# JaehaKim97/EDTR

Hardware: AMD Instinct MI355X
Metric: restored 512x512 images/sec @ 4 denoise steps (higher is better)
Workload: dtype bf16; 1 GPU; EDTR-det s4 (sd21): vae_encode + q_sample(t=200) + 4 x (ControlNet+UNet) + vae_decode, batch 8/GPU of 512x512; global_batch=8, image_size=512, denoise_steps=4, parallelism=batch-sharded x1, graphs=True, batches_in_flight=2, precision=fast

## Files before the change

### edtr_amd/build.py

```python
from __future__ import annotations

import os
import shutil
import subprocess
import sys

HERE = os.path.dirname(os.path.abspath(__file__))
CSRC = os.path.join(HERE, "csrc")
LIB_PATH = os.path.join(HERE, "libedtr_hip.so")
SOURCES = ["igemm.hip", "halo512.hip", "attention.hip", "attn512.hip", "norm.hip", "elementwise.hip", "swin.hip", "ffn.hip", "lin320.hip"]
HEADERS = [os.path.join(CSRC, "common.h"), os.path.join(os.path.dirname(HERE), "include", "edtr_hip.h")]
EXTRA_DEPS = {"attention.hip": [os.path.join(CSRC, "attn_v3_loop.inc")]}
ARCH = "gfx950"


def _hipcc() -> str:
    for cand in (os.environ.get("HIPCC"), shutil.which("hipcc"), "/opt/rocm/bin/hipcc"):
        if cand and os.path.exists(cand):
            return cand
    raise RuntimeError("hipcc not found (needed to build libedtr_hip.so)")


def _stale(target: str, deps) -> bool:
    if not os.path.exists(target):
        return True
    t = os.path.getmtime(target)
    return any(os.path.getmtime(d) > t for d in deps)


def source_hash() -> str:
    import hashlib
    h = hashlib.sha1()
    files = sorted(f for f in os.listdir(CSRC) if f.endswith((".hip", ".inc", ".h")))
# ... 62 lines not shown
```

### edtr_amd/engine.py

```python
from __future__ import annotations

import collections
import ctypes as ct
import math
import os
from dataclasses import dataclass
from typing import Dict, List, Optional, Sequence, Tuple

import torch

from . import lib as L
from . import ops
from .ops import Rec, round_up


class Arena:

    ALIGN = 256

    def __init__(self, device: torch.device, chunk_bytes: int = 1 << 28):
        self.device = device
        self.chunk_bytes = chunk_bytes
        self.chunks: List[torch.Tensor] = []
        self.free_lists: List[List[List[int]]] = []
# ... 235 lines not shown
            w1p, b1p, c1, c2 = self.ln_fold("geglu", [w1name], [b1name], ln_prefix)
            cst = ops.pack_ffn_constants(c2 + b1p)
            w2p = ops.pack_ffn_w2(self._p(w2name).reshape(self.params[w2name].shape[0], -1), self.dtype)
            self.cache[key] = (w1p, w2p, cst, self._p(b2name).reshape(-1).contiguous())
        return self.cache[key]

    def lin320(self, names: Sequence[str], biases, ln_prefix: Optional[str], alpha: float, vt_col0: Optional[int] = None, vt_alpha: float = 1.0):
        names = tuple(names)
        key = ("lin320", names, tuple(biases) if biases else None, ln_prefix, float(alpha), vt_col0, float(vt_alpha))
        if key not in self.cache:
            w = torch.cat([self._p(n).reshape(self.params[n].shape[0], -1) for n in names], dim=0)
            cvec = None
            if biases:
                cvec = torch.cat([self._p(bn).reshape(-1) if bn else torch.zeros(self.params[n].shape[0], device=self.device)
                                  for n, bn in zip(names, biases)]).float()
            if ln_prefix is not None:
                gamma, beta = self._p(ln_prefix + "weight").reshape(-1), self._p(ln_prefix + "bias").reshape(-1)
                shift = float(alpha) * (w @ beta)
                if vt_col0 is not None:
                    shift[vt_col0:] *= float(vt_alpha) / float(alpha)
                cvec = shift if cvec is None else cvec + shift
                w = w * gamma[None, :]
            self.cache[key] = (ops.pack_lin320_w(w, self.dtype), cvec.contiguous() if cvec is not None else None)
        return self.cache[key]

    def raw(self, name: str) -> torch.Tensor:
        key = ("raw", name)
        if key not in self.cache:
            self.cache[key] = self._p(name).contiguous()
        return self.cache[key]

    def geglu(self, wname: str, bname: str):
        n, k = self.shape_of(wname)[0], self.shape_of(wname)[1]

        def build(parts):
            w = self._p(wname)
            perm = ops.geglu_perm(w.shape[0] // 2).to(self.device)
            return ops.pack_linear_weight(w[perm], self.dtype, parts=parts)

        ref = WRef(self, ("geglu", wname), build, (round_up(n, 8), round_up(k, 8)))
        key = ("geglu.bias", bname)
        if key not in self.cache:
            b = self._p(bname)
            self.cache[key] = b[ops.geglu_perm(b.shape[0] // 2).to(self.device)].contiguous()
        return ref, self.cache[key]

# ... 305 lines not shown
        y = self.arena.alloc((rows, C), dtype or self.attn_dtype)
        self.prog.add(ops.make_cast16(dtype=dtype or self.attn_dtype, src=x, rows=rows, C=C, dst=y))
        return y

    @staticmethod
    def _w(w, parts: int) -> torch.Tensor:
        return w.get(parts) if isinstance(w, WRef) else w

    def ln_fold_ok(self, C: int, B: int = 0) -> bool:
        if self.hp or C % 32 or self.invariant:
            return False
        mode = os.environ.get("EDTR_LN_FOLD", "auto")
        if mode in ("0", "1"):
            return mode == "1"
        return 0 < B <= ops.LN_FOLD_MAX_BATCH

    def _ln_kwargs(self, a, K: int, ln_vec):
        if a.C != K or ln_vec is None:
            raise ValueError("folded LayerNorm: the consumer needs K == C and the folded weight's (c1, c2)")
        return a.x, dict(ln_stats=a.stats, ln_C=a.C, ln_valid=a.c_valid, ln_eps=1e-5, ln_c1=ln_vec[0], ln_c2=ln_vec[1])

    def ffn_ok(self, rows: int, C: int) -> bool:
        return not self.hp and not self.invariant and ops.ffn_ok(rows, C, 4 * C)

    def lin320_ok(self, rows: int, N: int, K: int, ln: bool = False) -> bool:
        return not self.hp and not self.invariant and ops.lin320_ok(rows, N, K, ln)

    def lin320(self, x: torch.Tensor, rows: int, N: int, names, biases=None, *, ln_prefix: Optional[str] = None, alpha: float = 1.0,
               residual: Optional[torch.Tensor] = None, gn_table: Optional[torch.Tensor] = None, rows_per_image: int = 0,
               name: str = "lin320") -> torch.Tensor:
        self.last_gnp, self.last_row_stats, self.gnp_into_done = None, None, False
        w, cvec = self.store.lin320(names, biases, ln_prefix, alpha)
        out = self.new(rows, N)
        self.prog.add(ops.make_lin320(dtype=self.dtype, x=x, ldx=x.stride(0), M=rows, N=N, w=w, cvec=cvec, alpha=alpha, ln=ln_prefix is not None,
                                      eps=1e-5, residual=residual, ldr=residual.stride(0) if residual is not None else 0, out=out,
                                      ldo=out.stride(0), gn_table=gn_table, rows_per_image=rows_per_image, name=name))
        return out

    def qkv_lin320(self, x: torch.Tensor, names, *, B: int, N: int, C: int, ln_prefix: str, alpha: float, name: str = "attn1.qkv"):
        M = B * N
        w, cvec = self.store.lin320(names, None, ln_prefix, alpha, vt_col0=2 * C, vt_alpha=1.0)
        qk = self.arena.alloc((M, 2 * C), self.attn_dtype)
        vt = self.arena.alloc((B * C, N), self.attn_dtype)
        self.prog.add(ops.make_lin320(dtype=self.dtype, x=x, ldx=x.stride(0), M=M, N=3 * C, w=w, cvec=cvec, alpha=alpha, ln=True, eps=1e-5, out=qk,
                                      ldo=2 * C, vt_out=vt, vt_col0=2 * C, vt_ld=N, vt_alpha=1.0, rows_per_image=N, name=name))
        return qk, vt, N
# ... 459 lines not shown
```

### edtr_amd/lib.py

```python
from __future__ import annotations

import ctypes as C
import os
from typing import Optional

HERE = os.path.dirname(os.path.abspath(__file__))
LIB_PATH = os.environ.get("EDTR_AMD_LIB") or os.path.join(HERE, "libedtr_hip.so")

BF16, F16, F32_SPLIT, F32_H1, F32_H2, F32_H3 = 0, 1, 2, 3, 4, 5
ACT_NONE, ACT_GEGLU, ACT_SILU, ACT_GELU, ACT_LRELU = 0, 1, 2, 3, 4

DECLARED_SYMBOLS = [
    "edtr_abi_version", "edtr_error_string", "edtr_device_info", "edtr_igemm", "edtr_flash_attn64",
    "edtr_gn_stats", "edtr_gn_apply", "edtr_gn_finalize", "edtr_gn_table", "edtr_layernorm", "edtr_softmax_rows", "edtr_nchw_to_nhwc",
    "edtr_nhwc_to_nchw", "edtr_add", "edtr_timestep_embedding", "edtr_sampler_update", "edtr_axpby", "edtr_q_sample", "edtr_split3", "edtr_cast16",
    "edtr_tile_accumulate", "edtr_divide", "edtr_wavelet_level", "edtr_gn_pool", "edtr_copy3d_f32", "edtr_graph_begin", "edtr_graph_end", "edtr_graph_launch",
    "edtr_graph_destroy", "edtr_zero_bytes", "edtr_embed_tokens", "edtr_window_attn", "edtr_pixel_unshuffle", "edtr_swin_mlp", "edtr_swin_attn", "edtr_swin_layer", "edtr_conv64", "edtr_conv128_out",
    "edtr_split_operand", "edtr_sampler_update_indexed", "edtr_gaussian_sample", "edtr_add_mirror", "edtr_igemm_plan", "edtr_flash_attn512",
    "edtr_ffn", "edtr_ffn_plan", "edtr_add_stats", "edtr_lin320", "edtr_lin320_plan",
]


class IgemmParams(C.Structure):
    _fields_ = [
        ("dtype", C.c_int32), ("taps", C.c_int32), ("M", C.c_int32), ("N", C.c_int32), ("K", C.c_int32),
        ("n_valid", C.c_int32), ("Z", C.c_int32), ("zdiv", C.c_int32),
        ("a1", C.c_void_p), ("a2", C.c_void_p),
        ("C1", C.c_int32), ("C2", C.c_int32), ("ld1", C.c_int32), ("ld2", C.c_int32),
        ("a_zs_outer", C.c_int64), ("a_zs_inner", C.c_int64),
        ("IH", C.c_int32), ("IW", C.c_int32), ("OH", C.c_int32), ("OW", C.c_int32),
        ("stride", C.c_int32), ("pad_t", C.c_int32), ("pad_l", C.c_int32), ("upsample2x", C.c_int32),
        ("w", C.c_void_p), ("ldw", C.c_int32),
        ("w_zs_outer", C.c_int64), ("w_zs_inner", C.c_int64),
        ("alpha", C.c_float),
        ("bias_n", C.c_void_p), ("bias_m", C.c_void_p),
        ("rowvec", C.c_void_p), ("rowvec_ld", C.c_int32), ("rows_per_image", C.c_int32),
        ("act", C.c_int32),
        ("residual", C.c_void_p), ("ldr", C.c_int32),
        ("out", C.c_void_p), ("ldc", C.c_int32), ("out_f32", C.c_int32),
        ("o_zs_outer", C.c_int64), ("o_zs_inner", C.c_int64),
        ("tile", C.c_int32), ("splitk", C.c_int32),
        ("workspace", C.c_void_p), ("workspace_bytes", C.c_int64),
# ... 52 lines not shown


class FfnParams(C.Structure):
    _fields_ = [
        ("dtype", C.c_int32), ("M", C.c_int32), ("D", C.c_int32), ("H", C.c_int32),
        ("eps", C.c_float),
        ("x", C.c_void_p), ("ldx", C.c_int32),
        ("w1", C.c_void_p), ("w2", C.c_void_p),
        ("cst", C.c_void_p), ("b2", C.c_void_p),
        ("out", C.c_void_p), ("ldo", C.c_int32),
    ]


class Lin320Params(C.Structure):
    _fields_ = [
        ("dtype", C.c_int32), ("M", C.c_int32), ("N", C.c_int32), ("K", C.c_int32),
        ("ln", C.c_int32), ("eps", C.c_float), ("alpha", C.c_float),
        ("x", C.c_void_p), ("ldx", C.c_int32),
        ("w", C.c_void_p), ("cvec", C.c_void_p),
        ("residual", C.c_void_p), ("ldr", C.c_int32),
        ("out", C.c_void_p), ("ldo", C.c_int32),
        ("vt_out", C.c_void_p), ("vt_col0", C.c_int32), ("vt_ld", C.c_int32), ("vt_alpha", C.c_float), ("rows_per_image", C.c_int32),
        ("gn_table", C.c_void_p),
    ]


class SwinAttnParams(C.Structure):
    _fields_ = [
        ("dtype", C.c_int32), ("B", C.c_int32), ("H", C.c_int32), ("W", C.c_int32),
        ("heads", C.c_int32), ("head_dim", C.c_int32), ("shift", C.c_int32),
        ("C", C.c_int32), ("c_valid", C.c_int32),
        ("eps", C.c_float),
        ("x", C.c_void_p), ("ldx", C.c_int32),
        ("wqkv", C.c_void_p), ("wproj", C.c_void_p),
        ("c1", C.c_void_p), ("c2b", C.c_void_p), ("bproj", C.c_void_p),
        ("bias", C.c_void_p), ("labels", C.c_void_p),
        ("out", C.c_void_p), ("ldo", C.c_int32),
    ]


class Conv64Params(C.Structure):
    _fields_ = [
        ("dtype", C.c_int32), ("B", C.c_int32), ("H", C.c_int32), ("W", C.c_int32),
        ("upsample2x", C.c_int32),
        ("x", C.c_void_p), ("ldx", C.c_int32),
        ("w", C.c_void_p), ("bias", C.c_void_p),
# ... 74 lines not shown
    lib.edtr_copy3d_f32.argtypes = [vp, i64, i64, vp, i64, i64, i32, i32, i32, vp]
    lib.edtr_graph_begin.argtypes = [vp]
    lib.edtr_graph_end.argtypes = [vp, C.POINTER(vp)]
    lib.edtr_graph_launch.argtypes = [vp, vp]
    lib.edtr_graph_destroy.argtypes = [vp]
    for name in DECLARED_SYMBOLS:
        fn = getattr(lib, name)
        if name not in ("edtr_error_string",):
            fn.restype = i32
    lib.edtr_zero_bytes.argtypes = [vp, i64, vp]
    lib.edtr_embed_tokens.argtypes = [i32, vp, vp, vp, i32, i32, i32, i32, vp, i32, vp]
    lib.edtr_window_attn.argtypes = [C.POINTER(WindowAttnParams), vp]
    lib.edtr_pixel_unshuffle.argtypes = [i32, vp, i32, i32, i32, i32, i32, vp, f32, vp, i32, i32, vp]
    lib.edtr_swin_mlp.argtypes = [C.POINTER(SwinMlpParams), vp]
    lib.edtr_swin_attn.argtypes = [C.POINTER(SwinAttnParams), vp]
    lib.edtr_conv64.argtypes = [C.POINTER(Conv64Params), vp]
    lib.edtr_conv128_out.argtypes = [C.POINTER(Conv128OutParams), vp]
    lib.edtr_swin_layer.argtypes = [C.POINTER(SwinAttnParams), C.POINTER(SwinMlpParams), vp]
    lib.edtr_add_stats.argtypes = [i32, vp, i32, vp, i32, vp, i32, i64, i32, vp, i32, i32, vp]
    lib.edtr_ffn.argtypes = [C.POINTER(FfnParams), vp]
    lib.edtr_ffn_plan.argtypes = [C.POINTER(FfnParams)]
    lib.edtr_lin320.argtypes = [C.POINTER(Lin320Params), vp]
    lib.edtr_lin320_plan.argtypes = [C.POINTER(Lin320Params)]
    if lib.edtr_abi_version() != 10:
        raise RuntimeError("libedtr_hip.so ABI version mismatch")
    _lib = lib
    return lib


def check(code: int, what: str = "") -> None:
    if code != 0:
        msg = load().edtr_error_string(code).decode()
        raise RuntimeError(f"libedtr_hip {what} failed with code {code}: {msg}")
```

### edtr_amd/model/cldm.py

```python
from __future__ import annotations

import os
from typing import Dict, List, Optional, Set, Tuple

import torch
from torch import nn

from .. import arch, nets
from .. import ops as ops_mod
from ..engine import Act, Arena, Emitter, EngineCache, Program, WeightStore
from .clip import FrozenOpenCLIPEmbedder
from .params import ParamTree, params_fingerprint

_DTYPES = {"bf16": torch.bfloat16, "bfloat16": torch.bfloat16, "fp16": torch.float16, "float16": torch.float16}


def default_compute_dtype() -> torch.dtype:
    return _DTYPES[os.environ.get("EDTR_AMD_DTYPE", "bf16").lower()]


PRECISIONS = ("fast", "mixed", "high", "hybrid", "robust")

HYBRID_SECTIONS = {"cldm": "fast16", "vae.encode": "fast16", "vae.decode": "mixed"}
_SECTION_MODES = {"fast16": ("fast", torch.float16), "fastbf16": ("fast", torch.bfloat16), "mixed": ("mixed", None), "high": ("high", None)}
# ... 152 lines not shown


class CldmEngine:

    def __init__(self, owner: "ControlLDM", B: int, h: int, w: int, nctx: int):
        dev = owner._device()
        mode, dt = section_mode(owner.precision, owner.compute_dtype, "cldm")
        pol = _policy_for(owner, "cldm")
        self.B, self.h, self.w, self.nctx = B, h, w, nctx
        self.arena = Arena(dev)
        store = owner._store("cldm")
        ua, ca = owner.unet.arch, owner.controlnet.arch
        f32 = torch.float32
        self.x_in = torch.zeros((B, ua.in_channels, h, w), dtype=f32, device=dev)
        self.hint_in = torch.zeros((B, ca.hint_channels, h, w), dtype=f32, device=dev)
        self.t_in = torch.zeros((B,), dtype=torch.int64, device=dev)
        self.ctx_in = torch.zeros((B, nctx, ua.context_dim), dtype=f32, device=dev)
        self.eps_out = torch.zeros((B, ua.out_channels, h, w), dtype=f32, device=dev)
        self.ctx_key = None

        self.ctx_prog = Program("cldm.context")
        em = Emitter(self.ctx_prog, self.arena, store, dt, mode, pol)
        ctx16 = em.cast_flat(self.ctx_in, B * nctx * ua.context_dim).view(B * nctx, ua.context_dim)
        self.kv_c = nets.emit_context_kv(em, "controlnet.", ca, ctx16, B, nctx)
        self.kv_u = nets.emit_context_kv(em, "unet.", ua, ctx16, B, nctx)

        self.step_prog = Program("cldm.step")
        em = Emitter(self.step_prog, self.arena, store, dt, mode, pol)
        hw = h * w
        cin_c = ca.in_channels + ca.hint_channels
        x8c = em.new(B * hw, arch_round8(cin_c))
        em.to_nhwc(self.x_in, B, ca.in_channels, hw, x8c, coff=0)
        em.to_nhwc(self.hint_in, B, ca.hint_channels, hw, x8c, coff=ca.in_channels,
                   pad_to=arch_round8(cin_c) - ca.in_channels)
        x8u = em.new(B * hw, arch_round8(ua.in_channels))
        em.to_nhwc(self.x_in, B, ua.in_channels, hw, x8u, coff=0, pad_to=arch_round8(ua.in_channels))
        tab_c, offs_c = nets.emit_time_rows(em, "controlnet.", ca, self.t_in, B)
        tab_u, offs_u = nets.emit_time_rows(em, "unet.", ua, self.t_in, B)
        self.arena_cn = Arena(dev)
        em_cn = Emitter(self.step_prog, self.arena_cn, store, dt, mode, pol)
        self.step_prog.fork()
        self.step_prog.set_lane(1)
        ctrl = nets.emit_controlnet(em_cn, "controlnet.", ca, Act(x8c, B, h, w, x8c.shape[1]), tab_c, offs_c, self.kv_c,
                                    list(owner.control_scales))
        self.step_prog.set_lane(0)
        eps = nets.emit_unet(em, "unet.", ua, Act(x8u, B, h, w, x8u.shape[1]), tab_u, offs_u, self.kv_u, ctrl,
                             before_control=self.step_prog.join)
        em.to_nchw(eps, B, ua.out_channels, hw, self.eps_out)
# ... 377 lines not shown
```

### edtr_amd/nets.py

```python
from __future__ import annotations

import math
import os
from typing import Dict, List, Optional, Tuple

import torch

from . import lib as L
from . import ops
from .arch import Layer, UNetArch, VaeLayer
from .engine import Act, Emitter, LNRef, LNReg
from .ops import round_up


def emit_time_rows(em: Emitter, P: str, a: UNetArch, t_dev: torch.Tensor, B: int) -> Tuple[torch.Tensor, Dict[str, int]]:
    mc, ted = a.model_channels, a.model_channels * 4
    temb = em.new(B, mc)
    em.prog.add(ops.make_timestep_embedding(dtype=em.io, t=t_dev, B=B, dim=mc, out=temb, ld=mc))
    w0, b0 = em.store.linear([P + "time_embed.0.weight"], [P + "time_embed.0.bias"])
    h = em.gemm(temb, w0, B, ted, mc, bias=b0, act=L.ACT_SILU, name="time_embed.0")
    w2, b2 = em.store.linear([P + "time_embed.2.weight"], [P + "time_embed.2.bias"])
    semb = em.gemm(h, w2, B, ted, ted, bias=b2, act=L.ACT_SILU, name="time_embed.2")
    res = a.res_layers()
    wall, ball = em.store.linear([P + l.prefix + "emb_layers.1.weight" for l in res],
# ... 1 lines not shown
    total = wall.shape[0]
    table = em.gemm(semb, wall, B, total, ted, bias=ball, out_f32=True, name="emb_layers(all)")
    em.free(temb, h, semb)
    offs, o = {}, 0
    for l in res:
        offs[l.prefix] = o
        o += l.cout
    return table, offs


ATTN_PRESCALE = 1.4426950408889634 / math.sqrt(64.0)


class ContextKV:

    def __init__(self):
        self.k_all = None
        self.vt_all = None
        self.sumC = 0
        self.ldv = 0
        self.Nctx = 0
        self.split = 0
        self.offs: Dict[str, int] = {}


def emit_context_kv(em: Emitter, P: str, a: UNetArch, ctx16: torch.Tensor, B: int, Nctx: int) -> ContextKV:
    layers = a.attn_layers()
    kv = ContextKV()
    t = "transformer_blocks.0.attn2."
    wk, _ = em.store.linear([P + l.prefix + t + "to_k.weight" for l in layers])
    wv, _ = em.store.linear([P + l.prefix + t + "to_v.weight" for l in layers])
    kv.sumC, kv.Nctx = wk.shape[0], Nctx
    kv.split = em.attn_split
    kv.k_all = em.gemm(ctx16, wk, B * Nctx, kv.sumC, a.context_dim, name="ctx_k(all)", out16=kv.split < 1)
    kv.vt_all, kv.ldv = em.vt_gemm(wv, ctx16, B=B, Ntok=Nctx, Cin=a.context_dim, name="ctx_vT(all)", out16=kv.split < 2)
    if kv.k_all.dtype == torch.float32:
        k32 = kv.k_all
        kv.k_all = em.split16(k32, B * Nctx, kv.sumC) if kv.split >= 1 else em.to16(k32, B * Nctx, kv.sumC)
        em.free(k32)
    if kv.vt_all.dtype == torch.float32:
        v32 = kv.vt_all
        kv.vt_all = em.split16(v32, B * kv.sumC, kv.ldv) if kv.split >= 2 else em.to16(v32, B * kv.sumC, kv.ldv)
        em.free(v32)
    o = 0
    for l in layers:
        kv.offs[l.prefix] = o
        o += l.cout
    return kv


def emit_resblock(em: Emitter, P: str, l: Layer, x: Act, table: torch.Tensor, offs: Dict[str, int], out=None, mirror=False, gnp_into=None) -> Act:
    p = P + l.prefix
    n1 = em.group_norm(x, p + "in_layers.0.", 1e-5, True, feeds=("res.conv1",), conv_n=l.cout)
    h = em.conv(n1, p + "in_layers.2.", rowvec=table[:, offs[l.prefix]:], name="res.conv1", stats=True, feeds=("res.conv2",))
    em.free(n1)
    n2 = em.group_norm(h, p + "out_layers.0.", 1e-5, True, feeds=("res.conv2",), conv_n=l.cout, take=True)
    em.free(h)
    if l.cin != l.cout:
        skip = em.conv(x, p + "skip_connection.", taps=1, name="res.skip1x1").t
    else:
        skip = x.t
    y = em.conv(n2, p + "out_layers.3.", residual=skip, out=out, name="res.conv2", stats=out is None, mirror=mirror, gnp_into=gnp_into)
    into_done = em.gnp_into_done
    em.free(n2)
    if l.cin != l.cout:
        em.free(skip)
    em.gnp_into_done = into_done
    return y


# ... 59 lines not shown
        t = em.gemm(n.t, wi, rows, C, C, bias=bi, name="st.proj_in", row_stats=fold1)
    st = em.last_row_stats
    em.free(n)
    tb = p + "transformer_blocks.0."
    if (st is None and em.fused_qkv_ok(N, C) and em.lin320_ok(rows, 3 * C, C, ln=True) and N % 32 == 0 and em.attn_dtype == em.dtype
            and os.environ.get("EDTR_LIN320_QKV", "1") != "0"):
        l1 = LNReg(t, C, tb + "norm1.")
    else:
        l1 = em.layer_norm(t, rows, C, tb + "norm1.", feeds=("attn1.qkv",) if em.fused_qkv_ok(N, C) else ("attn1.qk", "attn1.vT"), stats=st)
    t1 = emit_attention_core(em, tb + "attn1.", l1, B, N, C, l.heads, None, t, row_stats=fold)
    st = em.last_row_stats
    em.free(l1, t)
    l2 = (LNReg(t1, C, tb + "norm2.") if (st is None and em.lin320_ok(rows, C, C, ln=True))
          else em.layer_norm(t1, rows, C, tb + "norm2.", feeds=("attn2.q",), stats=st))
    off = kv.offs[l.prefix]
    k_view = kv.k_all[:, off:off + C]
    k_lo = kv.k_all[:, kv.sumC + off:kv.sumC + off + C] if kv.split >= 1 else None
    ldv_all = kv.vt_all.stride(0)
    vt3 = kv.vt_all.view(B, kv.sumC, ldv_all)
    vt_view = vt3[:, off:off + C, :kv.ldv]
    vt_lo = vt3[:, off:off + C, kv.ldv:] if kv.split >= 2 else None
    ctx = (k_view, vt_view, kv.Nctx * kv.k_all.stride(0), kv.sumC * ldv_all, ldv_all, kv.Nctx, k_lo, vt_lo)
    fused_ff = em.ffn_ok(rows, C)
    t2 = emit_attention_core(em, tb + "attn2.", l2, B, N, C, l.heads, ctx, t1, row_stats=fold and not fused_ff)
    st = em.last_row_stats
    em.free(l2, t1)
    if fused_ff:
        t3 = em.ffn(t2, rows, C, tb)
        em.free(t2)
    else:
        l3 = em.layer_norm(t2, rows, C, tb + "norm3.", feeds=("ff.geglu",), stats=st)
        if isinstance(l3, LNRef):
            wg, bg, c1, c2 = em.store.ln_fold("geglu", [tb + "ff.net.0.proj.weight"], [tb + "ff.net.0.proj.bias"], l3.prefix)
            g = em.gemm(l3, wg, rows, 8 * C, C, bias=bg, act=L.ACT_GEGLU, name="ff.geglu", feeds="ff.out", ln_vec=(c1, c2))
        else:
            wg, bg = em.store.geglu(tb + "ff.net.0.proj.weight", tb + "ff.net.0.proj.bias")
            g = em.gemm(l3, wg, rows, 8 * C, C, bias=bg, act=L.ACT_GEGLU, name="ff.geglu", feeds="ff.out")
        em.free(l3)
        wf, bf = em.store.linear([tb + "ff.net.2.weight"], [tb + "ff.net.2.bias"])
        t3 = em.gemm(g, wf, rows, C, 4 * C, bias=bf, residual=t2, name="ff.out", feeds="st.proj_out" if em.branch16 else None)
        em.free(g, t2)
    wo, bo = em.store.linear([p + "proj_out.weight"], [p + "proj_out.bias"])
    y = em.gemm(t3, wo, rows, C, C, bias=bo, residual=x.t, out=out, name="st.proj_out", stats_hw=N if (out is None or gnp_into is not None) else 0,
                mirror=mirror, gnp_into=gnp_into if out is not None else None)
    into_done = em.gnp_into_done
    em.free(t3)
    em.gnp_into_done = into_done
# ... 293 lines not shown
```

### edtr_amd/ops.py

```python
from __future__ import annotations

import ctypes as ct
import os
from typing import Optional, Sequence, Tuple

import torch

from . import lib as L

F32S = "f32_split"
F32H = {1: "f32_h1", 2: "f32_h2", 3: "f32_h3"}
MIXED = "f32_mixed"
PARTS_2W = 4
_DT = {torch.bfloat16: L.BF16, torch.float16: L.F16, F32S: L.F32_SPLIT, F32H[1]: L.F32_H1, F32H[2]: L.F32_H2, F32H[3]: L.F32_H3}


def dt_code(dtype: torch.dtype) -> int:
    try:
        return _DT[dtype]
    except KeyError:
        raise TypeError(f"libedtr_hip stores activations as bfloat16 or float16, got {dtype}")


def stream_ptr() -> int:
# ... 281 lines not shown
def pack_lin320_w(w: torch.Tensor, dtype: torch.dtype) -> torch.Tensor:
    n, k = w.shape
    assert k == LIN320_K and n % 32 == 0
    w16 = w.to(dtype).reshape(n // 32, 32, k // 16, 2, 8)
    return w16.permute(0, 2, 3, 1, 4).contiguous().reshape(-1)


def make_lin320(*, dtype, x, ldx, M, N, w, cvec=None, alpha=1.0, ln=False, eps=1e-5, residual=None, ldr=0, out, ldo, vt_out=None, vt_col0=0,
                vt_ld=0, vt_alpha=1.0, rows_per_image=0, gn_table=None, name="lin320") -> Rec:
    p = L.Lin320Params()
    p.dtype, p.M, p.N, p.K, p.ln, p.eps, p.alpha = dt_code(dtype), M, N, LIN320_K, int(ln), eps, alpha
    p.x, p.ldx, p.w, p.cvec = ptr(x), ldx, ptr(w), ptr(cvec)
    p.residual, p.ldr, p.out, p.ldo = ptr(residual), ldr, ptr(out), ldo
    p.vt_out, p.vt_col0, p.vt_ld, p.vt_alpha, p.rows_per_image = ptr(vt_out), vt_col0, vt_ld, vt_alpha, rows_per_image
    p.gn_table = ptr(gn_table)
    flops = 2.0 * M * N * LIN320_K
    nbytes = 2.0 * M * (LIN320_K + N * (2 if residual is not None else 1)) + 2.0 * N * LIN320_K
    rec = Rec(L.load().edtr_lin320, (ct.byref(p),), (p, x, w, cvec, residual, out, vt_out, gn_table), name, flops, nbytes)
    rec.tag = (f"lin320 M{M} N{N}" + (" ln" if ln else "") + (" gnin" if gn_table is not None else "") + (" res" if residual is not None else "")
               + (" vT" if vt_out is not None else ""))
    return rec


def make_swin_layer(attn: Rec, mlp: Rec, name="swin.layer") -> Rec:
    pa, pm = attn.keep[0], mlp.keep[0]
    return Rec(L.load().edtr_swin_layer, (ct.byref(pa), ct.byref(pm)), (attn.keep, mlp.keep), name, attn.flops + mlp.flops,
               attn.bytes + mlp.bytes - 4.0 * pa.B * pa.H * pa.W * SWIN_MLP_C)


def pack_conv64_weight(w: torch.Tensor, dtype: torch.dtype) -> torch.Tensor:
    co, ci, kh, kw = w.shape
    assert (kh, kw) == (3, 3) and co <= 64 and ci <= 64
    full = torch.zeros((9, 64, 8, 8), dtype=torch.float32, device=w.device)
    full.reshape(9, 64, 64)[:, :co, :ci] = w.permute(2, 3, 0, 1).reshape(9, co, ci)
    n = torch.arange(64, device=w.device)[:, None]
    c = torch.arange(8, device=w.device)[None, :]
    img = torch.empty_like(full)
    img[:, n, c ^ ((n >> 1) & 7)] = full[:, n, c]
    return img.to(dtype).reshape(-1).contiguous()


def pack_conv128_out_weight(w: torch.Tensor, dtype: torch.dtype) -> torch.Tensor:
    co, ci, kh, kw = w.shape
    assert (kh, kw) == (3, 3) and co <= 32 and ci == 128
    full = torch.zeros((9, 32, 16, 8), dtype=torch.float32, device=w.device)
    full.reshape(9, 32, 128)[:, :co] = w.permute(2, 3, 0, 1).reshape(9, co, ci)
# ... 342 lines not shown
```

### include/edtr_hip.h

```cpp
#ifndef EDTR_HIP_H
#define EDTR_HIP_H

#include <stdint.h>

#ifdef __cplusplus
extern "C" {
#endif

#define EDTR_ABI_VERSION 10

enum edtr_dtype {
    EDTR_BF16 = 0, EDTR_F16 = 1,
    EDTR_F32_SPLIT = 2,
    EDTR_F32_H1 = 3, EDTR_F32_H2 = 4, EDTR_F32_H3 = 5
};

enum edtr_error {
    EDTR_OK = 0,
    EDTR_E_NULL = -1,
    EDTR_E_SHAPE = -2,
    EDTR_E_ALIGN = -3,
    EDTR_E_DTYPE = -4,
    EDTR_E_UNSUPPORTED = -5
};
// ... 145 lines not shown
    const float* cst; const float* b2;
    void* out; int32_t ldo;
} edtr_ffn_params;

int edtr_ffn(const edtr_ffn_params* p, edtr_stream_t stream);
int edtr_ffn_plan(const edtr_ffn_params* p);

typedef struct edtr_lin320_params {
    int32_t dtype;
    int32_t M, N, K;
    int32_t ln; float eps;
    float alpha;
    const void* x; int32_t ldx;
    const void* w;
    const float* cvec;
    const void* residual; int32_t ldr;
    void* out; int32_t ldo;
    void* vt_out; int32_t vt_col0; int32_t vt_ld; float vt_alpha; int32_t rows_per_image;
    const float* gn_table;
} edtr_lin320_params;

int edtr_lin320(const edtr_lin320_params* p, edtr_stream_t stream);
int edtr_lin320_plan(const edtr_lin320_params* p);

typedef struct edtr_conv64_params {
    int32_t dtype;
    int32_t B, H, W;
    int32_t upsample2x;
    const void* x; int32_t ldx;
    const void* w;
    const float* bias;
    int32_t act; float act_slope; float alpha;
    void* out; int32_t ldo;
    int32_t out_nchw_f32, n_valid;
} edtr_conv64_params;

int edtr_conv64(const edtr_conv64_params* p, edtr_stream_t stream);

typedef struct edtr_conv128_out_params {
    int32_t dtype;
    int32_t B, H, W;
    const void* x; int32_t ldx;
    const float* gn_table;
    const void* w;
    const float* bias;
    float alpha;
// ... 65 lines not shown
```

Before: 122.9 images/s.

## Fuse 320-channel cross-attention by folding Q/K and V/Wo into per-image matrices

Adds a fused cross-attention kernel for the 320-channel UNet level. Per image and head, the query projection (with the LayerNorm affine) is pre-multiplied with the context keys, and the context values with the output projection. The main kernel then does LayerNorm, score GEMM, softmax, output GEMM, bias and residual in one pass, streaming the folded matrices through an LDS ring. This removes the separate Q projection, attention and out-projection launches and their intermediate HBM traffic, at the cost of a small per-step fold kernel and somewhat more MFMA work per row.

```diff
diff --git a/edtr_amd/build.py b/edtr_amd/build.py
--- a/edtr_amd/build.py
+++ b/edtr_amd/build.py
@@ -8,7 +8,7 @@
 HERE = os.path.dirname(os.path.abspath(__file__))
 CSRC = os.path.join(HERE, "csrc")
 LIB_PATH = os.path.join(HERE, "libedtr_hip.so")
-SOURCES = ["igemm.hip", "halo512.hip", "attention.hip", "attn512.hip", "norm.hip", "elementwise.hip", "swin.hip", "ffn.hip", "lin320.hip"]
+SOURCES = ["igemm.hip", "halo512.hip", "attention.hip", "attn512.hip", "norm.hip", "elementwise.hip", "swin.hip", "ffn.hip", "lin320.hip", "xattn320.hip"]
 HEADERS = [os.path.join(CSRC, "common.h"), os.path.join(os.path.dirname(HERE), "include", "edtr_hip.h")]
 EXTRA_DEPS = {"attention.hip": [os.path.join(CSRC, "attn_v3_loop.inc")]}
 ARCH = "gfx950"
diff --git a/edtr_amd/csrc/xattn320.hip b/edtr_amd/csrc/xattn320.hip
--- /dev/null
+++ b/edtr_amd/csrc/xattn320.hip
@@ -0,0 +1,337 @@
+#include <math.h>
+#include "common.h"
+
+namespace {
+
+constexpr int XC = 320;
+constexpr int XKS = XC / 16;
+constexpr int XBM = 128;
+constexpr int XHEADS = 5;
+constexpr int XNKP = 96;
+constexpr int XFRAG = 1024;
+constexpr int XCHB = 20 * XFRAG;
+constexpr int XCH_HEAD = 6;
+constexpr int XNCH = XHEADS * XCH_HEAD;
+constexpr int64_t XIMGB = (int64_t)XNCH * XCHB;
+constexpr int XRING = 6;
+constexpr int X_CS = XRING * XCHB;
+constexpr int X_LDS = X_CS + XHEADS * XNKP * 4;
+constexpr int XOPITCH = 656;
+static_assert(XBM * XOPITCH <= X_CS && X_LDS <= 160 * 1024, "LDS budget");
+static_assert(XRING == 6, "xwait's counts assume four chunks in flight behind the one waited for");
+
+template <bool DRAIN>
+__device__ __forceinline__ void xwait(int younger) {
+    if constexpr (DRAIN) {
+        asm volatile("s_waitcnt vmcnt(0)" ::: "memory");
+    } else {
+        if (younger >= 4) asm volatile("s_waitcnt vmcnt(20)" ::: "memory");
+        else if (younger == 3) asm volatile("s_waitcnt vmcnt(15)" ::: "memory");
+        else if (younger == 2) asm volatile("s_waitcnt vmcnt(10)" ::: "memory");
+        else if (younger == 1) asm volatile("s_waitcnt vmcnt(5)" ::: "memory");
+        else asm volatile("s_waitcnt vmcnt(0)" ::: "memory");
+    }
+}
+
+__device__ __forceinline__ void pin_frags(U4 (&w)[4]) {
+    asm volatile("" : "+v"(w[0].x), "+v"(w[0].y), "+v"(w[0].z), "+v"(w[0].w), "+v"(w[1].x), "+v"(w[1].y), "+v"(w[1].z), "+v"(w[1].w),
+                      "+v"(w[2].x), "+v"(w[2].y), "+v"(w[2].z), "+v"(w[2].w), "+v"(w[3].x), "+v"(w[3].y), "+v"(w[3].z), "+v"(w[3].w));
+}
+
+template <typename T, bool DRAIN>
+__global__ void __launch_bounds__(256, 1) xattn320_kernel(const edtr_xattn320_params p) {
+    extern __shared__ __attribute__((aligned(16))) char smem[];
+    const int tid = threadIdx.x, lane = tid & 63, wave = __builtin_amdgcn_readfirstlane(tid >> 6);
+    const int l31 = lane & 31, lh = lane >> 5;
+    int wg = blockIdx.x;
+    const int nwg = gridDim.x;
+    if ((nwg & 7) == 0) wg = (wg & 7) * (nwg >> 3) + (wg >> 3);
+    const int mt = wg * XBM;
+    const int img = mt / p.rows_per_image;
+    const int m0 = mt + 32 * wave;
+    const uint32_t lds0 = __builtin_amdgcn_readfirstlane(lds_addr_of(smem));
+
+    const u32x4 srd = make_srd(static_cast<const char*>(p.ab) + (int64_t)img * XIMGB);
+    auto issue = [&](int c) {
+        const uint32_t slot = lds0 + (uint32_t)((c % XRING) * XCHB);
+#pragma unroll
+        for (int i = 0; i < 5; ++i)
+            dma16_buf((uint32_t)(lane * 16), srd, (uint32_t)(c * XCHB + (5 * wave + i) * XFRAG), slot + (5 * wave + i) * XFRAG);
+    };
+    auto step = [&](int c) {
+        xwait<DRAIN>(min(XRING - 2, XNCH - 1 - c));
+        asm volatile("s_waitcnt lgkmcnt(0)" ::: "memory");
+        __builtin_amdgcn_s_barrier();
+        asm volatile("" ::: "memory");
+        if (c + XRING - 1 < XNCH) issue(c + XRING - 1);
+    };
+
+    U4 xf[XKS];
+    {
+        const uint16_t* xr = static_cast<const uint16_t*>(p.x) + (int64_t)(m0 + l31) * p.ldx + 8 * lh;
+#pragma unroll
+        for (int s = 0; s < XKS; ++s) xf[s] = ldg16(xr + 16 * s);
+    }
+#pragma unroll
+    for (int c = 0; c < XRING - 1; ++c) issue(c);
+    if (tid < XHEADS * XNKP / 4)
+        *reinterpret_cast<f32x4*>(smem + X_CS + 16 * tid) = *reinterpret_cast<const f32x4*>(p.cs + (int64_t)img * XHEADS * XNKP + 4 * tid);
+    {
+        float s = 0.0f;
+#pragma unroll
+        for (int i = 0; i < XKS; ++i) {
+            float f[8];
+            unpack8<T>(xf[i], f);
+#pragma unroll
+            for (int j = 0; j < 8; ++j) s += f[j];
+        }
+        s += __shfl_xor(s, 32, 64);
+        const float mean = s * (1.0f / XC);
+        float q = 0.0f;
+#pragma unroll
+        for (int i = 0; i < XKS; ++i) {
+            float f[8];
+            unpack8<T>(xf[i], f);
+#pragma unroll
+            for (int j = 0; j < 8; ++j) { const float dlt = f[j] - mean; q = __builtin_fmaf(dlt, dlt, q); }
+        }
+        q += __shfl_xor(q, 32, 64);
+        const float rstd = __builtin_amdgcn_rsqf(q * (1.0f / XC) + p.eps);
+        const float shift = -mean * rstd;
+#pragma unroll
+        for (int i = 0; i < XKS; ++i) {
+            float f[8];
+            unpack8<T>(xf[i], f);
+#pragma unroll
+            for (int j = 0; j < 8; ++j) f[j] = __builtin_fmaf(f[j], rstd, shift);
+            xf[i] = pack8<T>(f);
+        }
+    }
+    asm volatile("s_waitcnt vmcnt(0) lgkmcnt(0)" ::: "memory");
+
+    f32x16 oacc[10];
+#pragma unroll
+    for (int b = 0; b < 10; ++b)
+#pragma unroll
+        for (int r = 0; r < 16; ++r) oacc[b][r] = 0.0f;
+
+#pragma unroll 1
+    for (int h = 0; h < XHEADS; ++h) {
+        f32x16 sc[3];
+#pragma unroll
+        for (int kt = 0; kt < 3; ++kt) {
+            const int c = XCH_HEAD * h + kt;
+            step(c);
+            const char* wb = smem + (c % XRING) * XCHB + lane * 16;
+            f32x16 a;
+#pragma unroll
+            for (int r = 0; r < 16; ++r) a[r] = 0.0f;
+#pragma unroll
+            for (int s = 0; s < XKS; s += 4) {
+                U4 w[4];
+#pragma unroll
+                for (int i = 0; i < 4; ++i) w[i] = *reinterpret_cast<const U4*>(wb + (s + i) * XFRAG);
+                pin_frags(w);
+#pragma unroll
+                for (int i = 0; i < 4; ++i) a = T::mfma(w[i], xf[s + i], a);
+            }
+            sc[kt] = a;
+        }
+        U4 pf[6];
+        {
+            const float* cr = reinterpret_cast<const float*>(smem + X_CS) + h * XNKP + 4 * lh;
+            float mx = -INFINITY;
+#pragma unroll
+            for (int kt = 0; kt < 3; ++kt)
+#pragma unroll
+                for (int j = 0; j < 4; ++j) {
+                    const f32x4 cv = *reinterpret_cast<const f32x4*>(cr + 32 * kt + 8 * j);
+#pragma unroll
+                    for (int e = 0; e < 4; ++e) {
+                        sc[kt][4 * j + e] += cv[e];
+                        mx = fmaxf(mx, sc[kt][4 * j + e]);
+                    }
+                }
+            mx = fmaxf(mx, __shfl_xor(mx, 32, 64));
+            float sum = 0.0f;
+#pragma unroll
+            for (int kt = 0; kt < 3; ++kt)
+#pragma unroll
+                for (int r = 0; r < 16; ++r) {
+                    sc[kt][r] = __builtin_amdgcn_exp2f(sc[kt][r] - mx);
+                    sum += sc[kt][r];
+                }
+            sum += __shfl_xor(sum, 32, 64);
+            const float inv = __builtin_amdgcn_rcpf(sum);
+#pragma unroll
+            for (int kt = 0; kt < 3; ++kt)
+#pragma unroll
+                for (int jj = 0; jj < 2; ++jj) {
+                    float f[8];
+#pragma unroll
+                    for (int e = 0; e < 8; ++e) f[e] = sc[kt][8 * jj + e] * inv;
+                    pf[2 * kt + jj] = pack8<T>(f);
+                }
+        }
+#pragma unroll
+        for (int j = 0; j < 3; ++j) {
+            const int c = XCH_HEAD * h + 3 + j;
+            step(c);
+            const char* wb = smem + (c % XRING) * XCHB + lane * 16;
+#pragma unroll
+            for (int nt = 0; nt < 10; nt += 2) {
+                U4 w[4];
+#pragma unroll
+                for (int i = 0; i < 4; ++i) w[i] = *reinterpret_cast<const U4*>(wb + (2 * nt + i) * XFRAG);
+                pin_frags(w);
+#pragma unroll
+                for (int i = 0; i < 4; ++i) oacc[nt + (i >> 1)] = T::mfma(w[i], pf[2 * j + (i & 1)], oacc[nt + (i >> 1)]);
+            }
+        }
+    }
+
+    asm volatile("s_waitcnt lgkmcnt(0)" ::: "memory");
+    __builtin_amdgcn_s_barrier();
+    asm volatile("" ::: "memory");
+    {
+        const uint16_t* xr = static_cast<const uint16_t*>(p.x) + (int64_t)(m0 + l31) * p.ldx;
+        char* trow = smem + (32 * wave + l31) * XOPITCH;
+#pragma unroll
+        for (int nt = 0; nt < 10; ++nt) {
+            uint2 res[4];
+#pragma unroll
+            for (int q = 0; q < 4; ++q) res[q] = *reinterpret_cast<const uint2*>(xr + 32 * nt + 8 * q + 4 * lh);
+#pragma unroll
+            for (int q = 0; q < 4; ++q) {
+                const int n = 32 * nt + 8 * q + 4 * lh;
+                const f32x4 bias = *reinterpret_cast<const f32x4*>(p.bias + n);
+                const float r0 = T::to_f32((uint16_t)(res[q].x & 0xffff)), r1 = T::to_f32((uint16_t)(res[q].x >> 16));
+                const float r2 = T::to_f32((uint16_t)(res[q].y & 0xffff)), r3 = T::to_f32((uint16_t)(res[q].y >> 16));
+                uint2 o;
+                o.x = pack2<T>(oacc[nt][4 * q + 0] + bias[0] + r0, oacc[nt][4 * q + 1] + bias[1] + r1);
+                o.y = pack2<T>(oacc[nt][4 * q + 2] + bias[2] + r2, oacc[nt][4 * q + 3] + bias[3] + r3);
+                *reinterpret_cast<uint2*>(trow + n * 2) = o;
+            }
+        }
+    }
+    __syncthreads();
+    {
+        uint16_t* og = static_cast<uint16_t*>(p.out);
+#pragma unroll
+        for (int i = 0; i < (XBM * 40) / 256; ++i) {
+            const int idx = tid + 256 * i, row = idx / 40, ch = idx - row * 40;
+            const U4 v = *reinterpret_cast<const U4*>(smem + row * XOPITCH + ch * 16);
+            stg16(og + (int64_t)(mt + row) * p.ldo + ch * 8, v);
+        }
+    }
+}
+
+constexpr int XFOLD_FRAGS = XCH_HEAD * 20 + 1;
+
+template <typename T>
+__global__ void __launch_bounds__(64) xattn320_fold_kernel(const edtr_xattn320_fold_params p) {
+    const int lane = threadIdx.x, l31 = lane & 31, lh = lane >> 5;
+    const int f = blockIdx.x % XFOLD_FRAGS, bh = blockIdx.x / XFOLD_FRAGS;
+    const int h = bh % XHEADS, b = bh / XHEADS;
+    const uint16_t* kb = static_cast<const uint16_t*>(p.k) + (int64_t)b * p.k_bs + 64 * h;
+    const uint16_t* vb = static_cast<const uint16_t*>(p.vt) + (int64_t)b * p.vt_bs + (int64_t)(64 * h) * p.vt_ld;
+    if (f == XFOLD_FRAGS - 1) {
+        for (int key = lane; key < XNKP; key += 64) {
+            float acc = -INFINITY;
+            if (key < p.nctx) {
+                acc = 0.0f;
+                for (int d = 0; d < 64; ++d) acc = __builtin_fmaf(p.qb[64 * h + d], T::to_f32(kb[(int64_t)key * p.k_ld + d]), acc);
+            }
+            p.cs[(int64_t)bh * XNKP + key] = acc;
+        }
+        return;
+    }
+    float acc[8];
+#pragma unroll
+    for (int e = 0; e < 8; ++e) acc[e] = 0.0f;
+    if (f < 60) {
+        const int kt = f / 20, s = f - 20 * kt, key = 32 * kt + l31, k0 = 16 * s + 8 * lh;
+        if (key < p.nctx) {
+            for (int d = 0; d < 64; ++d) {
+                const float kv = T::to_f32(kb[(int64_t)key * p.k_ld + d]);
+                const float* wr = p.wq + (int64_t)(64 * h + d) * XC + k0;
+#pragma unroll
+                for (int e = 0; e < 8; ++e) acc[e] = __builtin_fmaf(wr[e], kv, acc[e]);
+            }
+        }
+    } else {
+        constexpr int perm[16] = {0, 1, 2, 3, 8, 9, 10, 11, 4, 5, 6, 7, 12, 13, 14, 15};
+        const int g = f - 60, j = g / 20, nt = (g - 20 * j) >> 1, u = g & 1, n = 32 * nt + l31;
+        int keys[8];
+#pragma unroll
+        for (int e = 0; e < 8; ++e) keys[e] = 32 * j + 16 * u + perm[8 * lh + e];
+        for (int d = 0; d < 64; ++d) {
+            const float w = p.wo[(int64_t)n * XC + 64 * h + d];
+            const uint16_t* vr = vb + (int64_t)d * p.vt_ld;
+#pragma unroll
+            for (int e = 0; e < 8; ++e)
+                if (keys[e] < p.nctx) acc[e] = __builtin_fmaf(T::to_f32(vr[keys[e]]), w, acc[e]);
+        }
+    }
+    stg16(static_cast<char*>(p.ab) + ((int64_t)bh * (XFOLD_FRAGS - 1) + f) * XFRAG + lane * 16, pack8<T>(acc));
+}
+
+int check_xattn320(const edtr_xattn320_params& p) {
+    if (!p.x || !p.ab || !p.cs || !p.bias || !p.out) return EDTR_E_NULL;
+    if (p.dtype != EDTR_BF16 && p.dtype != EDTR_F16) return EDTR_E_DTYPE;
+    if (p.M <= 0 || p.rows_per_image <= 0 || p.nctx <= 0) return EDTR_E_SHAPE;
+    if (p.C != XC || p.heads != XHEADS || p.nctx > XNKP) return EDTR_E_UNSUPPORTED;
+    if ((p.M % XBM) || (p.rows_per_image % XBM) || (p.M % p.rows_per_image)) return EDTR_E_UNSUPPORTED;
+    if (p.ldx < XC || p.ldo < XC) return EDTR_E_SHAPE;
+    if ((p.ldx & 7) || (p.ldo & 7)) return EDTR_E_ALIGN;
+    if (!aligned16(p.x) || !aligned16(p.ab) || !aligned16(p.cs) || !aligned16(p.bias) || !aligned16(p.out)) return EDTR_E_ALIGN;
+    if (p.x == p.out) return EDTR_E_UNSUPPORTED;
+    return EDTR_OK;
+}
+
+int check_fold(const edtr_xattn320_fold_params& p) {
+    if (!p.wq || !p.qb || !p.wo || !p.k || !p.vt || !p.ab || !p.cs) return EDTR_E_NULL;
+    if (p.dtype != EDTR_BF16 && p.dtype != EDTR_F16) return EDTR_E_DTYPE;
+    if (p.B <= 0 || p.nctx <= 0) return EDTR_E_SHAPE;
+    if (p.C != XC || p.heads != XHEADS || p.nctx > XNKP) return EDTR_E_UNSUPPORTED;
+    if (p.k_ld < XC || p.vt_ld < p.nctx || p.k_bs < (int64_t)p.nctx * p.k_ld || p.vt_bs < (int64_t)XC * p.vt_ld) return EDTR_E_SHAPE;
+    if (!aligned16(p.ab) || !aligned16(p.cs)) return EDTR_E_ALIGN;
+    return EDTR_OK;
+}
+
+template <typename T>
+int launch_xattn320(const edtr_xattn320_params& p, hipStream_t stream) {
+    static EdtrLdsOnce once[2];
+    auto go = [&](auto kern, EdtrLdsOnce& o) -> int {
+        if (int rc_ = edtr_lds_attr(reinterpret_cast<const void*>(kern), X_LDS, o)) return rc_;
+        hipLaunchKernelGGL(kern, dim3((unsigned)(p.M / XBM)), dim3(256), X_LDS, stream, p);
+        EDTR_LAUNCH_CHECK();
+        return EDTR_OK;
+    };
+    return p.drain ? go(&xattn320_kernel<T, true>, once[1]) : go(&xattn320_kernel<T, false>, once[0]);
+}
+
+}
+
+extern "C" int edtr_xattn320(const edtr_xattn320_params* pp, edtr_stream_t stream) {
+    if (!pp) return EDTR_E_NULL;
+    if (int e = check_xattn320(*pp)) return e;
+    hipStream_t s = static_cast<hipStream_t>(stream);
+    return pp->dtype == EDTR_BF16 ? launch_xattn320<BF16>(*pp, s) : launch_xattn320<F16>(*pp, s);
+}
+
+extern "C" int edtr_xattn320_plan(const edtr_xattn320_params* pp) {
+    if (!pp) return EDTR_E_NULL;
+    return check_xattn320(*pp);
+}
+
+extern "C" int edtr_xattn320_fold(const edtr_xattn320_fold_params* pp, edtr_stream_t stream) {
+    if (!pp) return EDTR_E_NULL;
+    if (int e = check_fold(*pp)) return e;
+    hipStream_t s = static_cast<hipStream_t>(stream);
+    const dim3 grid((unsigned)(pp->B * XHEADS * XFOLD_FRAGS)), block(64);
+    if (pp->dtype == EDTR_BF16) hipLaunchKernelGGL(xattn320_fold_kernel<BF16>, grid, block, 0, s, *pp);
+    else hipLaunchKernelGGL(xattn320_fold_kernel<F16>, grid, block, 0, s, *pp);
+    EDTR_LAUNCH_CHECK();
+    return EDTR_OK;
+}
diff --git a/edtr_amd/engine.py b/edtr_amd/engine.py
--- a/edtr_amd/engine.py
+++ b/edtr_amd/engine.py
@@ -281,6 +281,17 @@
                 cvec = shift if cvec is None else cvec + shift
                 w = w * gamma[None, :]
             self.cache[key] = (ops.pack_lin320_w(w, self.dtype), cvec.contiguous() if cvec is not None else None)
+        return self.cache[key]
+
+    def xattn320(self, p: str, ln_prefix: str, scale: float):
+        key = ("xattn320", p, ln_prefix, float(scale))
+        if key not in self.cache:
+            wq = self._p(p + "to_q.weight").float()
+            wq = wq.reshape(wq.shape[0], -1)
+            gamma, beta = self._p(ln_prefix + "weight").reshape(-1).float(), self._p(ln_prefix + "bias").reshape(-1).float()
+            wo = self._p(p + "to_out.0.weight").float()
+            self.cache[key] = ((float(scale) * wq * gamma[None, :]).contiguous(), (float(scale) * (wq @ beta)).contiguous(),
+                               wo.reshape(wo.shape[0], -1).contiguous(), self._p(p + "to_out.0.bias").reshape(-1).float().contiguous())
         return self.cache[key]
 
     def raw(self, name: str) -> torch.Tensor:
@@ -632,6 +643,17 @@
 
     def ffn_ok(self, rows: int, C: int) -> bool:
         return not self.hp and not self.invariant and ops.ffn_ok(rows, C, 4 * C)
+
+    def xattn320_ok(self, rows: int, C: int, heads: int, nctx: int, rows_per_image: int) -> bool:
+        return not self.hp and not self.invariant and ops.xattn320_ok(rows, C, heads, nctx, rows_per_image)
+
+    def xattn320(self, x: torch.Tensor, rows: int, C: int, xa, nctx: int, rows_per_image: int, name: str = "attn2.fused") -> torch.Tensor:
+        ab, cs, bo = xa
+        self.last_gnp, self.last_row_stats, self.gnp_into_done = None, None, False
+        out = self.new(rows, C)
+        self.prog.add(ops.make_xattn320(dtype=self.dtype, x=x, ldx=x.stride(0), M=rows, nctx=nctx, rows_per_image=rows_per_image, ab=ab, cs=cs,
+                                        bias=bo, out=out, ldo=out.stride(0), name=name))
+        return out
 
     def lin320_ok(self, rows: int, N: int, K: int, ln: bool = False) -> bool:
         return not self.hp and not self.invariant and ops.lin320_ok(rows, N, K, ln)
diff --git a/edtr_amd/lib.py b/edtr_amd/lib.py
--- a/edtr_amd/lib.py
+++ b/edtr_amd/lib.py
@@ -18,6 +18,7 @@
     "edtr_graph_destroy", "edtr_zero_bytes", "edtr_embed_tokens", "edtr_window_attn", "edtr_pixel_unshuffle", "edtr_swin_mlp", "edtr_swin_attn", "edtr_swin_layer", "edtr_conv64", "edtr_conv128_out",
     "edtr_split_operand", "edtr_sampler_update_indexed", "edtr_gaussian_sample", "edtr_add_mirror", "edtr_igemm_plan", "edtr_flash_attn512",
     "edtr_ffn", "edtr_ffn_plan", "edtr_add_stats", "edtr_lin320", "edtr_lin320_plan",
+    "edtr_xattn320", "edtr_xattn320_plan", "edtr_xattn320_fold",
 ]
 
 
@@ -116,6 +117,28 @@
         ("out", C.c_void_p), ("ldo", C.c_int32),
         ("vt_out", C.c_void_p), ("vt_col0", C.c_int32), ("vt_ld", C.c_int32), ("vt_alpha", C.c_float), ("rows_per_image", C.c_int32),
         ("gn_table", C.c_void_p),
+    ]
+
+
+class Xattn320Params(C.Structure):
+    _fields_ = [
+        ("dtype", C.c_int32), ("M", C.c_int32), ("C", C.c_int32), ("heads", C.c_int32), ("nctx", C.c_int32), ("rows_per_image", C.c_int32),
+        ("eps", C.c_float),
+        ("x", C.c_void_p), ("ldx", C.c_int32),
+        ("ab", C.c_void_p), ("cs", C.c_void_p),
+        ("bias", C.c_void_p),
+        ("out", C.c_void_p), ("ldo", C.c_int32),
+        ("drain", C.c_int32),
+    ]
+
+
+class Xattn320FoldParams(C.Structure):
+    _fields_ = [
+        ("dtype", C.c_int32), ("B", C.c_int32), ("C", C.c_int32), ("heads", C.c_int32), ("nctx", C.c_int32),
+        ("wq", C.c_void_p), ("qb", C.c_void_p), ("wo", C.c_void_p),
+        ("k", C.c_void_p), ("k_bs", C.c_int64), ("k_ld", C.c_int32),
+        ("vt", C.c_void_p), ("vt_bs", C.c_int64), ("vt_ld", C.c_int32),
+        ("ab", C.c_void_p), ("cs", C.c_void_p),
     ]
 
 
@@ -236,6 +259,9 @@
     lib.edtr_ffn_plan.argtypes = [C.POINTER(FfnParams)]
     lib.edtr_lin320.argtypes = [C.POINTER(Lin320Params), vp]
     lib.edtr_lin320_plan.argtypes = [C.POINTER(Lin320Params)]
+    lib.edtr_xattn320.argtypes = [C.POINTER(Xattn320Params), vp]
+    lib.edtr_xattn320_plan.argtypes = [C.POINTER(Xattn320Params)]
+    lib.edtr_xattn320_fold.argtypes = [C.POINTER(Xattn320FoldParams), vp]
     if lib.edtr_abi_version() != 10:
         raise RuntimeError("libedtr_hip.so ABI version mismatch")
     _lib = lib
diff --git a/edtr_amd/model/cldm.py b/edtr_amd/model/cldm.py
--- a/edtr_amd/model/cldm.py
+++ b/edtr_amd/model/cldm.py
@@ -198,8 +198,8 @@
         self.ctx_prog = Program("cldm.context")
         em = Emitter(self.ctx_prog, self.arena, store, dt, mode, pol)
         ctx16 = em.cast_flat(self.ctx_in, B * nctx * ua.context_dim).view(B * nctx, ua.context_dim)
-        self.kv_c = nets.emit_context_kv(em, "controlnet.", ca, ctx16, B, nctx)
-        self.kv_u = nets.emit_context_kv(em, "unet.", ua, ctx16, B, nctx)
+        self.kv_c = nets.emit_context_kv(em, "controlnet.", ca, ctx16, B, nctx, hw=h * w)
+        self.kv_u = nets.emit_context_kv(em, "unet.", ua, ctx16, B, nctx, hw=h * w)
 
         self.step_prog = Program("cldm.step")
         em = Emitter(self.step_prog, self.arena, store, dt, mode, pol)
diff --git a/edtr_amd/nets.py b/edtr_amd/nets.py
--- a/edtr_amd/nets.py
+++ b/edtr_amd/nets.py
@@ -47,9 +47,11 @@
         self.Nctx = 0
         self.split = 0
         self.offs: Dict[str, int] = {}
-
-
-def emit_context_kv(em: Emitter, P: str, a: UNetArch, ctx16: torch.Tensor, B: int, Nctx: int) -> ContextKV:
+        self.xa: Dict[str, Tuple[torch.Tensor, torch.Tensor, torch.Tensor]] = {}
+        self.hw = 0
+
+
+def emit_context_kv(em: Emitter, P: str, a: UNetArch, ctx16: torch.Tensor, B: int, Nctx: int, hw: int = 0) -> ContextKV:
     layers = a.attn_layers()
     kv = ContextKV()
     t = "transformer_blocks.0.attn2."
@@ -71,6 +73,22 @@
     for l in layers:
         kv.offs[l.prefix] = o
         o += l.cout
+    kv.hw = hw
+    if hw and kv.split == 0 and kv.k_all.dtype == em.dtype and kv.vt_all.dtype == em.dtype:
+        ldk, ldv_all = kv.k_all.stride(0), kv.vt_all.stride(0)
+        vt3 = kv.vt_all.view(B, kv.sumC, ldv_all)
+        for l in layers:
+            if not em.xattn320_ok(B * hw, l.cout, l.heads, Nctx, hw):
+                continue
+            tb = P + l.prefix + "transformer_blocks.0."
+            wq, qb, wo, bo = em.store.xattn320(tb + "attn2.", tb + "norm2.", ATTN_PRESCALE)
+            off = kv.offs[l.prefix]
+            ab = em.arena.alloc((B * ops.XATTN_IMG_ELEMS,), em.dtype)
+            cs = em.arena.alloc((B * ops.XATTN_HEADS * ops.XATTN_NKP,), torch.float32)
+            em.prog.add(ops.make_xattn320_fold(dtype=em.dtype, B=B, nctx=Nctx, wq=wq, qb=qb, wo=wo, k=kv.k_all[:, off:off + l.cout],
+                                               k_bs=Nctx * ldk, k_ld=ldk, vt=vt3[:, off:off + l.cout, :], vt_bs=kv.sumC * ldv_all,
+                                               vt_ld=ldv_all, ab=ab, cs=cs, name="attn2.fold"))
+            kv.xa[l.prefix] = (ab, cs, bo)
     return kv
 
 
@@ -176,7 +194,11 @@
     vt_lo = vt3[:, off:off + C, kv.ldv:] if kv.split >= 2 else None
     ctx = (k_view, vt_view, kv.Nctx * kv.k_all.stride(0), kv.sumC * ldv_all, ldv_all, kv.Nctx, k_lo, vt_lo)
     fused_ff = em.ffn_ok(rows, C)
-    t2 = emit_attention_core(em, tb + "attn2.", l2, B, N, C, l.heads, ctx, t1, row_stats=fold and not fused_ff)
+    xa = kv.xa.get(l.prefix) if N == kv.hw else None
+    if xa is not None and isinstance(l2, LNReg) and not (fold and not fused_ff):
+        t2 = em.xattn320(t1, rows, C, xa, kv.Nctx, N)
+    else:
+        t2 = emit_attention_core(em, tb + "attn2.", l2, B, N, C, l.heads, ctx, t1, row_stats=fold and not fused_ff)
     st = em.last_row_stats
     em.free(l2, t1)
     if fused_ff:
diff --git a/edtr_amd/ops.py b/edtr_amd/ops.py
--- a/edtr_amd/ops.py
+++ b/edtr_amd/ops.py
@@ -327,6 +327,98 @@
     return rec
 
 
+XATTN_C, XATTN_HEADS, XATTN_NKP, XATTN_ROWS = 320, 5, 96, 128
+XATTN_IMG_ELEMS = XATTN_HEADS * 6 * 20 * 64 * 8
+
+
+def device_cus() -> int:
+    try:
+        if torch.cuda.is_available():
+            return int(torch.cuda.get_device_properties(torch.cuda.current_device()).multi_processor_count)
+    except Exception:
+        pass
+    return 256
+
+
+def xattn320_ok(M: int, C: int, heads: int, nctx: int, rows_per_image: int) -> bool:
+    if os.environ.get("EDTR_XATTN320", "1") == "0" or C != XATTN_C or heads != XATTN_HEADS or not 0 < nctx <= XATTN_NKP:
+        return False
+    if M <= 0 or rows_per_image <= 0 or rows_per_image % XATTN_ROWS or M % rows_per_image:
+        return False
+    env = os.environ.get("EDTR_XATTN320_MIN_ROWS")
+    return M >= (int(env) if env else XATTN_ROWS * device_cus())
+
+
+def xattn320_fold_ref(wq, wk_ctx, vt_ctx, wo, gamma, beta, scale: float):
+    wq, k, vt, wo = (torch.as_tensor(t).double() for t in (wq, wk_ctx, vt_ctx, wo))
+    gamma, beta = torch.as_tensor(gamma).double(), torch.as_tensor(beta).double()
+    A, cs, B = [], [], []
+    for h in range(XATTN_HEADS):
+        d = slice(64 * h, 64 * h + 64)
+        a = scale * wq[d].t() @ k[:, d].t()
+        A.append(gamma[:, None] * a)
+        cs.append(beta @ a)
+        B.append(vt[d].t() @ wo[:, d].t())
+    return torch.stack(A), torch.stack(cs), torch.stack(B)
+
+
+def _xattn_index(nctx: int):
+    ch, f, lane, e = torch.meshgrid(torch.arange(6), torch.arange(20), torch.arange(64), torch.arange(8), indexing="ij")
+    l31, lh = lane % 32, lane // 32
+    is_a = ch < 3
+    perm = torch.tensor(FFN_PERM16)[8 * lh + e]
+    a_key, a_k = 32 * ch + l31, 16 * f + 8 * lh + e
+    b_key, b_n = 32 * (ch - 3) + 16 * (f % 2) + perm, 32 * (f // 2) + l31
+    row = torch.where(is_a, a_k, b_key)
+    col = torch.where(is_a, a_key, b_n)
+    return is_a.reshape(-1), row.reshape(-1), col.reshape(-1)
+
+
+def xattn320_pack_ref(A, B, dtype) -> torch.Tensor:
+    A, B = torch.as_tensor(A).double(), torch.as_tensor(B).double()
+    nctx = A.shape[2]
+    Ap = torch.nn.functional.pad(A, (0, XATTN_NKP - nctx))
+    Bp = torch.nn.functional.pad(B, (0, 0, 0, XATTN_NKP - nctx))
+    is_a, row, col = _xattn_index(nctx)
+    out = torch.empty(XATTN_HEADS, is_a.numel(), dtype=torch.float64)
+    for h in range(XATTN_HEADS):
+        out[h] = torch.where(is_a, Ap[h][row, col.clamp_max(XATTN_NKP - 1)], Bp[h][row.clamp_max(XATTN_NKP - 1), col.clamp_max(XATTN_C - 1)])
+    return out.to(dtype).reshape(-1)
+
+
+def xattn320_unpack(stream, nctx: int):
+    s = torch.as_tensor(stream).double().reshape(XATTN_HEADS, -1)
+    is_a, row, col = _xattn_index(nctx)
+    A = torch.zeros(XATTN_HEADS, XATTN_C, XATTN_NKP, dtype=torch.float64)
+    B = torch.zeros(XATTN_HEADS, XATTN_NKP, XATTN_C, dtype=torch.float64)
+    for h in range(XATTN_HEADS):
+        A[h][row[is_a], col[is_a]] = s[h][is_a]
+        B[h][row[~is_a], col[~is_a]] = s[h][~is_a]
+    return A[:, :, :nctx], B[:, :nctx, :], torch.cat([A[:, :, nctx:].reshape(-1), B[:, nctx:, :].reshape(-1)])
+
+
+def make_xattn320(*, dtype, x, ldx, M, nctx, rows_per_image, ab, cs, bias, out, ldo, eps=1e-5, drain=False, name="attn2.fused") -> Rec:
+    p = L.Xattn320Params()
+    p.dtype, p.M, p.C, p.heads, p.nctx, p.rows_per_image, p.eps = dt_code(dtype), M, XATTN_C, XATTN_HEADS, nctx, rows_per_image, eps
+    p.x, p.ldx, p.ab, p.cs, p.bias, p.out, p.ldo, p.drain = ptr(x), ldx, ptr(ab), ptr(cs), ptr(bias), ptr(out), ldo, int(drain)
+    flops = 2.0 * M * XATTN_HEADS * 2 * XATTN_C * XATTN_NKP
+    nbytes = 2.0 * M * 2 * XATTN_C + 2.0 * (M // rows_per_image) * XATTN_IMG_ELEMS
+    rec = Rec(L.load().edtr_xattn320, (ct.byref(p),), (p, x, ab, cs, bias, out), name, flops, nbytes)
+    rec.tag = f"xattn320 M{M} Nk{nctx}"
+    return rec
+
+
+def make_xattn320_fold(*, dtype, B, nctx, wq, qb, wo, k, k_bs, k_ld, vt, vt_bs, vt_ld, ab, cs, name="attn2.fold") -> Rec:
+    p = L.Xattn320FoldParams()
+    p.dtype, p.B, p.C, p.heads, p.nctx = dt_code(dtype), B, XATTN_C, XATTN_HEADS, nctx
+    p.wq, p.qb, p.wo, p.k, p.k_bs, p.k_ld = ptr(wq), ptr(qb), ptr(wo), ptr(k), k_bs, k_ld
+    p.vt, p.vt_bs, p.vt_ld, p.ab, p.cs = ptr(vt), vt_bs, vt_ld, ptr(ab), ptr(cs)
+    rec = Rec(L.load().edtr_xattn320_fold, (ct.byref(p),), (p, wq, qb, wo, k, vt, ab, cs), name, 2.0 * B * XATTN_HEADS * 2 * 64 * XATTN_C * XATTN_NKP,
+              2.0 * B * XATTN_IMG_ELEMS)
+    rec.tag = f"xattn320.fold B{B} Nk{nctx}"
+    return rec
+
+
 def make_swin_layer(attn: Rec, mlp: Rec, name="swin.layer") -> Rec:
     pa, pm = attn.keep[0], mlp.keep[0]
     return Rec(L.load().edtr_swin_layer, (ct.byref(pa), ct.byref(pm)), (attn.keep, mlp.keep), name, attn.flops + mlp.flops,
diff --git a/include/edtr_hip.h b/include/edtr_hip.h
--- a/include/edtr_hip.h
+++ b/include/edtr_hip.h
@@ -191,6 +191,30 @@
 
 int edtr_lin320(const edtr_lin320_params* p, edtr_stream_t stream);
 int edtr_lin320_plan(const edtr_lin320_params* p);
+
+typedef struct edtr_xattn320_params {
+    int32_t dtype;
+    int32_t M, C, heads, nctx, rows_per_image;
+    float eps;
+    const void* x; int32_t ldx;
+    const void* ab; const float* cs;
+    const float* bias;
+    void* out; int32_t ldo;
+    int32_t drain;
+} edtr_xattn320_params;
+
+typedef struct edtr_xattn320_fold_params {
+    int32_t dtype;
+    int32_t B, C, heads, nctx;
+    const float* wq; const float* qb; const float* wo;
+    const void* k; int64_t k_bs; int32_t k_ld;
+    const void* vt; int64_t vt_bs; int32_t vt_ld;
+    void* ab; float* cs;
+} edtr_xattn320_fold_params;
+
+int edtr_xattn320(const edtr_xattn320_params* p, edtr_stream_t stream);
+int edtr_xattn320_plan(const edtr_xattn320_params* p);
+int edtr_xattn320_fold(const edtr_xattn320_fold_params* p, edtr_stream_t stream);
 
 typedef struct edtr_conv64_params {
     int32_t dtype;
```

Result: no change. 123.4 images/s (median of 6 runs) (+0.4%).
